# jolideco/jolideco

Hardware: AMD Instinct MI355X
Metric: MAP iters/sec at 2048x2048, 8-obs joint fit (higher is better)
Workload: dtype f32; 1 GPU; c3: 2048x2048, 8 observations (Gaussian PSFs sigma = 1.5 + 0.25 i on 6 x 17x17 + 2 x 33x33, varying exposure/background), GMM patch prior 8x8 stride 4 K=128, joint fit, Adam lr 0.1; global_observations=8, conv_method=separable

## Files before the change

### jolideco_amd/csrc/gmm_screen.hip

```cpp
#include "gmm_internal.h"

namespace jd {

struct __attribute__((packed, aligned(4))) F4U {
  float x, y, z, w;
};

__global__ __launch_bounds__(256) void gmm_stage_kernel(GmmStageArgs a) {
  use_device_shift(a);
  if (a.pcount && blockIdx.x == 0 && threadIdx.x == 0) *a.dense_count = 0;
  const int lane = threadIdx.x & 63;
  const int tile = blockIdx.x * 4 + (threadIdx.x >> 6);
  if (tile >= a.n_tiles) return;
  const int h = lane >> 5, c = lane & 31;
  const int n = a.n_begin + 32 * tile + c;
  const bool valid = n < a.n_end;
  const int py = valid ? n / a.nPx : 0, px = valid ? n - (n / a.nPx) * a.nPx : 0;
  const int x0 = px * a.stride - a.shift_x;
  const int xb = x0 < 0 ? x0 + a.W : x0;
  const bool straight = xb + 7 < a.W;
  float x[32];
#pragma unroll
  for (int s = 0; s < 4; ++s) {
    const float* row = a.flux + (size_t)wrap(py * a.stride + 2 * s + h - a.shift_y, a.H) * a.W;
// ... 192 lines not shown
    pL[p] = -INFINITY;
    pq[p] = 0.f;
    pc[p] = 0;
    okm[p] = __ballot(pok[p]);
  }

  ScreenFrags f0, f1;
  f32x16 acc[2][2][2];
  auto issue_pair = [&](f32x16 (&buf)[2][2], const ScreenFrags& f, int p) {
#pragma unroll
    for (int u = 0; u < 2; ++u) {
      mfma_screen(buf[u], f, xf[2 * p + u]);
    }
  };
  constexpr int KSTEP = KSPLIT ? 4 : 1;
  const int kk0 = KSPLIT ? wave : 0;
  struct KConst {
    int k;
    float ck, ef, sk2, mn, ack;
  };
  auto fetch_consts = [&](int pos) {
    KConst r;
    if (KC_LDS) {
      r.k = kc_k[pos];
      const float4 c4 = kc_f[pos];
      r.ck = c4.x, r.ef = c4.y, r.sk2 = c4.z, r.mn = c4.w, r.ack = kc_a[pos];
    } else {
      r.k = a.korder[pos];
      r.ck = a.const_k[r.k], r.ef = a.efro_k[r.k], r.sk2 = a.sk2_k[r.k], r.mn = a.mnorm_k[r.k];
      r.ack = fmaf(1e-6f, fabsf(r.ck), 1e-30f);
    }
    return r;
  };
  auto clamp_pos = [&](int pos) { return pos < a.K ? pos : (kk0 < a.K ? kk0 : 0); };
  auto fetch_k = [&](int pos) { return KC_LDS ? kc_k[pos] : a.korder[pos]; };
  KConst cur = fetch_consts(clamp_pos(kk0));
  KConst nxt = fetch_consts(clamp_pos(kk0 + KSTEP));
  load_frags16(f0, af, __builtin_amdgcn_readfirstlane(cur.k));
  load_frags16(f1, af, __builtin_amdgcn_readfirstlane(nxt.k));
  issue_pair(acc[0], f0, 0);
  int k_ahead_next = fetch_k(clamp_pos(kk0 + 2 * KSTEP));
  auto component = [&](ScreenFrags& fa, const ScreenFrags& fb, int kk, auto phase, bool live) {
    constexpr int PHASE = decltype(phase)::value;
    const int k = __builtin_amdgcn_readfirstlane(cur.k);
    const float ck = cur.ck, ef = cur.ef, sk2 = cur.sk2, mn = cur.mn;
    const float ack = cur.ack;
    const int k_ahead = k_ahead_next;
    k_ahead_next = fetch_k(clamp_pos(kk + 3 * KSTEP));
    cur = nxt;
    nxt = fetch_consts(clamp_pos(kk + 2 * KSTEP));
    unsigned long long m0 = 0ull, m1 = 0ull;
    float u0 = 0.f, u1 = 0.f;
    if (NP == 2) {
      issue_pair(acc[1], fa, 1);
      load_frags16(fa, af, __builtin_amdgcn_readfirstlane(k_ahead));
      screen_finish_pair<LSE>(acc[0][0], acc[0][1], ck, ack, mn, ef, pxn[0], ps2[0] * sk2, pok[0], pL[0], pq[0], pc[0], keep,
                              m0, u0, live ? okm[0] : 0ull, live);
      issue_pair(acc[0], fb, 0);
      screen_finish_pair<LSE>(acc[1][0], acc[1][1], ck, ack, mn, ef, pxn[NP - 1], ps2[NP - 1] * sk2, pok[NP - 1], pL[NP - 1],
                              pq[NP - 1], pc[NP - 1], keep, m1, u1, live ? okm[NP - 1] : 0ull, live);
    } else {
      load_frags16(fa, af, __builtin_amdgcn_readfirstlane(k_ahead));
      issue_pair(acc[1 - PHASE], fb, 0);
      screen_finish_pair<LSE>(acc[PHASE][0], acc[PHASE][1], ck, ack, mn, ef, pxn[0], ps2[0] * sk2, pok[0], pL[0], pq[0], pc[0],
                              keep, m0, u0, live ? okm[0] : 0ull, live);
    }
    if (NP == 2 && !LSE && !KSPLIT) {
#pragma unroll
      for (int i = 0; i < 12 * NP; ++i) {
        __builtin_amdgcn_sched_group_barrier(0x008, 1, 0);
        __builtin_amdgcn_sched_group_barrier(0x002, 8, 0);
      }
    }
    if (m0 | m1) {
      screen_emit(m0, u0, pn[0], k, lane, cnt_l, lb_n, lb_k, lb_ub, SCREEN_RB);
      if (NP == 2) screen_emit(m1, u1, pn[NP - 1], k, lane, cnt_l, lb_n, lb_k, lb_ub, SCREEN_RB);
      flush(false);
    }
  };
  for (int kk = kk0; kk < a.K; kk += 2 * KSTEP) {
    component(f0, f1, kk, std::integral_constant<int, 0>{}, true);
    component(f1, f0, kk + KSTEP, std::integral_constant<int, 1>{}, kk + KSTEP < a.K);
  }
  bool trouble = false;
#pragma unroll
  for (int p = 0; p < NP; ++p) {
    trouble = trouble || (pok[p] && !(pq[p] < 3.0e38f));
    if (LSE && pc[p] > keep && pn[p] < a.n_end) a.dense_mark[pn[p]] = 1;
    if (KSPLIT)
      st_L[wave * (NT * 32) + (2 * p + h) * 32 + c] = pL[p];
    else if (pn[p] < a.n_end)
      a.lfinal[pn[p]] = pL[p];
  }
  if (KSPLIT) {
    __syncthreads();
    for (int i = threadIdx.x; i < NT * 32; i += 256)
      if (base + i < a.n_end)
        a.lfinal[base + i] = fmaxf(fmaxf(st_L[i], st_L[NT * 32 + i]), fmaxf(st_L[2 * NT * 32 + i], st_L[3 * NT * 32 + i]));
  }
  flush(true);
  if (lane == 0) a.seg_cnt[wave_global] = cnt < SCREEN_CAP ? cnt : SCREEN_CAP;
  if (__ballot(trouble) != 0ull || cnt > SCREEN_CAP) {
    if (lane == 0) __hip_atomic_store(a.flag, a.gen, __ATOMIC_RELAXED, __HIP_MEMORY_SCOPE_AGENT);
  }
  if (CLOCK) {
    __syncthreads();
    if (threadIdx.x == 0 && (int)blockIdx.x < a.clock_cap) {
      a.clock_stamps[2 * blockIdx.x] = __builtin_amdgcn_s_memtime() - clock_t0;
      a.clock_stamps[2 * blockIdx.x + 1] = __builtin_amdgcn_s_memrealtime() - clock_r0;
    }
  }
}

#ifdef JD_EXACT_STAMPS
#define EXACT_STAMP(i)                                                              \
  do {                                                                              \
    __builtin_amdgcn_sched_barrier(0);                                              \
    const unsigned long long t_ = __builtin_amdgcn_s_memtime();                     \
    __builtin_amdgcn_sched_barrier(0);                                              \
    if (lane == 0) a.stamps[(size_t)grp * 8 + (i)] = t_;                            \
  } while (0)
#else
#define EXACT_STAMP(i) do {} while (0)
#endif

constexpr int EXACT_PITCH = 68;
constexpr int EXACT_DRAW = 1;
constexpr int EXACT_OFF_LDS = 1025;

template <bool TRI>
__global__ __launch_bounds__(256) void gmm_exact_kernel(GmmExactArgs a) {
  use_device_shift(a);
  if (*a.flag == a.gen) return;
  __shared__ __attribute__((aligned(16))) float stage[4][32 * EXACT_PITCH];
  const int lane = threadIdx.x & 63, wave = threadIdx.x >> 6;
  const int g = lane >> 4, n16 = lane & 15;
  const int wave_global = blockIdx.x * 4 + wave;
  const int n_waves = gridDim.x * 4;
  const int n_groups = a.offsets[a.K] >> 5;
  float* st = stage[wave];
  (void)n_waves, (void)wave_global;
  __shared__ int s_off[EXACT_OFF_LDS];
  __shared__ int s_next;
  const bool off_lds = a.K + 1 <= EXACT_OFF_LDS;
  const int per_block = (n_groups + (int)gridDim.x - 1) / (int)gridDim.x;
  const int b_begin = (int)blockIdx.x * per_block, b_end = b_begin + per_block < n_groups ? b_begin + per_block : n_groups;
  if (threadIdx.x == 0) s_next = b_begin;
  if (off_lds)
    for (int i = threadIdx.x; i <= a.K; i += 256) s_off[i] = a.offsets[i];
  __syncthreads();
  auto offset_of = [&](int kk) { return off_lds ? s_off[kk] : a.offsets[kk]; };
  int k = -1;
  float ck = 0.f;
  float4 A[4][4], M[4];
  for (;;) {
    int g_begin = 0;
    if (lane == 0) g_begin = atomicAdd(&s_next, EXACT_DRAW);
    g_begin = __builtin_amdgcn_readfirstlane(g_begin);
    if (g_begin >= b_end) break;
    const int g_end = g_begin + EXACT_DRAW < b_end ? g_begin + EXACT_DRAW : b_end;
  for (int grp = g_begin; grp < g_end; ++grp) {
    EXACT_STAMP(0);
    int kg = k;
    if (kg < 0 || offset_of(kg) > 32 * grp || offset_of(kg + 1) <= 32 * grp) {
      int lo = 0, hi = a.K;
      while (hi - lo > 1) {
        const int mid = (lo + hi) >> 1;
        if (offset_of(mid) <= 32 * grp) lo = mid; else hi = mid;
      }
      kg = lo;
    }
    if (kg != k) {
      k = kg;
      ck = a.const_k[k];
      const float4* ak = reinterpret_cast<const float4*>(a.afrag) + (size_t)k * (AFRAG_FLOATS / 4) + lane;
      const float4* mk = reinterpret_cast<const float4*>(a.mfrag) + (size_t)k * 16 + g;
#pragma unroll
      for (int jb = 0; jb < 4; ++jb) {
        M[jb] = mk[jb * 4];
#pragma unroll
        for (int st4 = 0; st4 < 4; ++st4)
          if (!TRI || st4 <= jb) A[jb][st4] = ak[(jb * 4 + st4) * 64];
      }
    }
    const int nvalid = a.counts[k] - (32 * grp - offset_of(k));
#ifdef JD_EXACT_STAMPS
    if (lane == 0) a.stamps[(size_t)grp * 8 + 7] = (unsigned long long)((nvalid << 8) | (k & 255));
    { float touch = A[0][0].x + M[0].x; asm volatile("" ::"v"(touch)); }
#endif
    EXACT_STAMP(1);
    {
      const int q = lane >> 1, hh = lane & 1;
      const bool have = q < nvalid;
      const int n = have ? a.order_n[32 * grp + q] : 0;
      const int py = n / a.nPx, px = n - py * a.nPx;
      const int x0 = px * a.stride + 4 * hh - a.shift_x;
      const bool straight = x0 >= 0 && x0 + 3 < a.W;
      const int xw[4] = {wrap(x0, a.W), wrap(x0 + 1, a.W), wrap(x0 + 2, a.W), wrap(x0 + 3, a.W)};
      float4 rows[8];
#pragma unroll
      for (int r = 0; r < 8; ++r) {
        const float* row = a.flux + (size_t)wrap(py * a.stride + r - a.shift_y, a.H) * a.W;
        if (straight) {
          const F4U v = *reinterpret_cast<const F4U*>(row + x0);
          rows[r] = make_float4(v.x, v.y, v.z, v.w);
        } else {
          rows[r] = make_float4(row[xw[0]], row[xw[1]], row[xw[2]], row[xw[3]]);
        }
      }
#pragma unroll
      for (int r = 0; r < 8; ++r) *reinterpret_cast<float4*>(st + q * EXACT_PITCH + 8 * r + 4 * hh) = rows[r];
    }
    EXACT_STAMP(2);
    int n[2];
    bool valid[2];
    float x[2][16];
#pragma unroll
    for (int nb = 0; nb < 2; ++nb) {
      const int q = 16 * nb + n16;
      valid[nb] = q < nvalid;
      n[nb] = valid[nb] ? a.order_n[32 * grp + q] : 0;
#pragma unroll
      for (int s4 = 0; s4 < 16; ++s4) x[nb][s4] = valid[nb] ? st[q * EXACT_PITCH + 4 * s4 + g] : 0.f;
      const float mean = patch_mean_groups(x[nb]);
#pragma unroll
      for (int s4 = 0; s4 < 16; ++s4) x[nb][s4] -= mean;
    }
#ifdef JD_EXACT_STAMPS
    { float touch = x[0][0] + x[1][15]; asm volatile("" ::"v"(touch)); }
#endif
    EXACT_STAMP(3);
    f32x4 y[4][2];
#pragma unroll
    for (int jb = 0; jb < 4; ++jb) {
      y[jb][0] = y[jb][1] = f32x4{M[jb].x, M[jb].y, M[jb].z, M[jb].w};
#pragma unroll
      for (int st4 = 0; st4 < 4; ++st4) {
        if (TRI && st4 > jb) continue;
#pragma unroll
        for (int e = 0; e < 4; ++e)
#pragma unroll
          for (int nb = 0; nb < 2; ++nb)
            y[jb][nb] = __builtin_amdgcn_mfma_f32_16x16x4f32(f4_get(A[jb][st4], e), x[nb][4 * st4 + e], y[jb][nb], 0, 0, 0);
      }
    }
#ifdef JD_EXACT_STAMPS
    { float touch = y[3][1][3] + y[0][0][0]; asm volatile("" ::"v"(touch)); }
#endif
    EXACT_STAMP(4);
#pragma unroll
    for (int nb = 0; nb < 2; ++nb) {
      const float l = fmaf(-0.5f, sum_lane_groups(sum_squares(y, nb)), ck);
      const int tie = a.grec ? 32 * grp + 16 * nb + n16 : k;
      if (a.lrec) {
        if (g == 0 && valid[nb]) a.lrec[32 * grp + 16 * nb + n16] = l;
      } else if (g == 0 && valid[nb] && l > -INFINITY) {
        atomicMax(a.best + n[nb], best_key(l, tie));
      }
    }
    EXACT_STAMP(5);
    if (a.grec) {
      float* rows[2] = {a.grec + (size_t)(32 * grp + n16) * D, a.grec + (size_t)(32 * grp + 16 + n16) * D};
      patch_gradient_rows<TRI>(y, a.gfrag, k, lane, valid, rows);
    }
#ifdef JD_EXACT_STAMPS
    __builtin_amdgcn_s_waitcnt(0);
#endif
    EXACT_STAMP(6);
  }
  }
}

constexpr int BEST_CHUNK = 1024;

__global__ __launch_bounds__(256) void gmm_best_kernel(GmmBestArgs a) {
  use_device_shift(a.fb);
  __shared__ double red[4];
  const int base = a.n_begin + blockIdx.x * BEST_CHUNK;
  const bool slots = a.winner && *a.flag != a.gen;
  double local = 0.0;
  unsigned long long keys[BEST_CHUNK / 256];
#pragma unroll
  for (int i = 0; i < BEST_CHUNK / 256; ++i) {
    const int n = base + i * 256 + threadIdx.x;
    keys[i] = a.best[n < a.n_end ? n : a.n_end - 1];
  }
  if (slots && !a.argmax_out) {
#pragma unroll
    for (int i = 0; i < BEST_CHUNK / 256; ++i) {
      const int n = base + i * 256 + threadIdx.x;
      if (n < a.n_end) {
        const unsigned long long key = keys[i];
        const bool ok = key != 0ull;
        const float v = best_value(key);
        a.winner[n] = ok && v > -INFINITY ? best_component(key) : -1;
        if (ok) local += (double)v;
      }
    }
  } else
#pragma unroll
  for (int i = 0; i < BEST_CHUNK / 256; ++i) {
    const int n = base + i * 256 + threadIdx.x;
    if (n < a.n_end) {
      const unsigned long long key = keys[i];
      const bool ok = key != 0ull;
      const float v = best_value(key);
      int k = ok ? best_component(key) : -1;
      if (slots) {
        const int slot = ok && v > -INFINITY ? k : -1;
        a.winner[n] = slot;
        if (a.argmax_out) k = ok ? (slot >= 0 ? a.rec_k[a.rec_order[slot]] : 0) : -1;
      } else if (a.argmax_fb) {
        a.argmax_fb[n] = k;
      }
      if (a.argmax_out) a.argmax_out[n] = k;
      if (ok) local += (double)v;
    }
  }
  local = wave_sum(local);
  if ((threadIdx.x & 63) == 0) red[threadIdx.x >> 6] = local;
  __syncthreads();
  if (a.fb.gpatch && !slots && a.winner) {
    __syncthreads();
    const int grp0 = blockIdx.x * (BEST_CHUNK / 32);
    const int n_groups = (a.n_end - a.n_begin + 31) >> 5;
    const int grp1 = grp0 + BEST_CHUNK / 32 < n_groups ? grp0 + BEST_CHUNK / 32 : n_groups;
    bwd_fallback_groups<true>(a.fb, grp0 + (threadIdx.x >> 6), grp1, 4);
  }
  __shared__ int last;
  if (threadIdx.x == 0) {
    a.partials[blockIdx.x] = (red[0] + red[1]) + (red[2] + red[3]);
    __threadfence();
    last = atomicAdd(a.ticket, 1) == (int)gridDim.x - 1 ? 1 : 0;
  }
  __syncthreads();
  if (!last) return;
  __threadfence();
  __shared__ double smem[4];
  double acc = 0.0;
  for (int i = threadIdx.x; i < (int)gridDim.x; i += 256) {
    const unsigned long long bits = __hip_atomic_load(reinterpret_cast<const unsigned long long*>(a.partials + i),
                                                      __ATOMIC_RELAXED, __HIP_MEMORY_SCOPE_AGENT);
    acc += __builtin_bit_cast(double, bits);
  }
  const double total = block_sum<256>(acc, smem);
  if (threadIdx.x == 0) {
    double v = a.scale * total;
    if (a.accumulate) v += (double)a.value_out[0];
    a.value_out[0] = (float)v;
    *a.ticket = 0;
    if (a.host_stats) {
      a.host_stats[1] = *a.flag == a.gen ? 1 : 0;
      a.host_stats[2] = *a.slots_used;
      a.host_stats[3] = a.n_end - a.n_begin;
      __threadfence_system();
      a.host_stats[0] = a.gen;
    }
  }
}

constexpr int LSE_ROWS = 32;

__global__ __launch_bounds__(256) void gmm_lse_combine_kernel(GmmLseCombineArgs a) {
  __shared__ int s_slot[16][LSE_ROWS];
  __shared__ float s_l[16][LSE_ROWS];
  if (*a.flag == a.gen) return;
  const int grp = threadIdx.x >> 4, part = threadIdx.x & 15;
  const int n = a.n_begin + (int)blockIdx.x * 16 + grp;
  const bool live = n < a.n_end && a.mark[n < a.n_end ? n : a.n_begin] == 0;
  int c = live ? a.pcount[n] : 0;
  if (c > a.rows) c = a.rows;
  int slot[2];
  float l[2];
#pragma unroll
  for (int u = 0; u < 2; ++u) {
    const int j = part + 16 * u;
    slot[u] = j < c ? a.ptab[(size_t)n * a.rows + j] : 0x7fffffff;
    l[u] = j < c ? a.lrec[slot[u]] : -INFINITY;
  }
  int rank[2] = {0, 0};
  for (int j = 0; j < c; ++j) {
    const int other = __shfl(j < 16 ? slot[0] : slot[1], (threadIdx.x & 48) + (j & 15), 64);
    rank[0] += other < slot[0] ? 1 : 0;
    rank[1] += other < slot[1] ? 1 : 0;
  }
#pragma unroll
  for (int u = 0; u < 2; ++u)
    if (part + 16 * u < c) s_slot[grp][rank[u]] = slot[u], s_l[grp][rank[u]] = l[u];
  float m = fmaxf(l[0], l[1]);
#pragma unroll
  for (int o = 8; o >= 1; o >>= 1) m = fmaxf(m, __shfl_xor(m, o, 64));
  __syncthreads();
  float4 G = make_float4(0.f, 0.f, 0.f, 0.f);
  float S = 0.f;
  for (int r = 0; r < c; ++r) {
    const float e = expf(s_l[grp][r] - m);
    const float4 row = reinterpret_cast<const float4*>(a.grec + (size_t)s_slot[grp][r] * D)[part];
    S += e;
    G.x = fmaf(e, row.x, G.x), G.y = fmaf(e, row.y, G.y), G.z = fmaf(e, row.z, G.z), G.w = fmaf(e, row.w, G.w);
  }
  if (live) {
    const float inv = c > 0 ? 1.f / S : 0.f;
    reinterpret_cast<float4*>(a.gpatch + (size_t)(n - a.n_begin) * D)[part] = make_float4(G.x * inv, G.y * inv, G.z * inv, G.w * inv);
  }
  if (part == 0 && live) a.vpatch[n] = c > 0 ? m + logf(S) : 0.f;
}

__global__ __launch_bounds__(256) void gmm_lse_list_kernel(const int* mark, int n_begin, int n_end, const int* flag, int gen,
                                                           int32_t* list, int* count) {
  __shared__ int wave_cnt[4][4];
  __shared__ int base;
  if (*flag == gen) return;
  const int lane = threadIdx.x & 63, wave = threadIdx.x >> 6;
  const int first = n_begin + (int)blockIdx.x * 1024;
  bool marked[4];
  int rank[4];
#pragma unroll
  for (int i = 0; i < 4; ++i) {
    const int n = first + i * 256 + (int)threadIdx.x;
    marked[i] = n < n_end && mark[n] != 0;
    const unsigned long long b = __ballot(marked[i]);
    rank[i] = __popcll(b & ((1ull << lane) - 1ull));
    if (lane == 0) wave_cnt[i][wave] = __popcll(b);
  }
  __syncthreads();
  if (threadIdx.x == 0) {
    int total = 0;
#pragma unroll
    for (int i = 0; i < 4; ++i)
#pragma unroll
      for (int w = 0; w < 4; ++w) {
        const int c = wave_cnt[i][w];
        wave_cnt[i][w] = total;
        total += c;
      }
    base = total ? atomicAdd(count, total) : 0;
  }
  __syncthreads();
#pragma unroll
  for (int i = 0; i < 4; ++i)
    if (marked[i]) list[base + wave_cnt[i][wave] + rank[i]] = first + i * 256 + (int)threadIdx.x;
}

__global__ __launch_bounds__(256) void gmm_lse_value_kernel(const float* vpatch, const int* mark, int n_begin, int n_end,
                                                            double* partials, int* marked) {
  __shared__ double red[4];
  __shared__ int redm[4];
  const int base = n_begin + (int)blockIdx.x * 1024;
  double local = 0.0;
  int cnt = 0;
#pragma unroll
  for (int i = 0; i < 4; ++i) {
    const int n = base + i * 256 + (int)threadIdx.x;
    const bool marked = n < n_end && mark[n] != 0;
    if (n < n_end) local += (double)vpatch[n];
    cnt += __popcll(__ballot(marked));
  }
  local = wave_sum(local);
  if ((threadIdx.x & 63) == 0) red[threadIdx.x >> 6] = local, redm[threadIdx.x >> 6] = cnt;
  __syncthreads();
  if (threadIdx.x == 0) {
    partials[blockIdx.x] = (red[0] + red[1]) + (red[2] + red[3]);
    marked[blockIdx.x] = (redm[0] + redm[1]) + (redm[2] + redm[3]);
  }
}

__global__ __launch_bounds__(256) void gmm_lse_finalize_kernel(const double* partials, const int* marked, int count,
                                                               const int* flag, int gen, double scale, float* value_out,
                                                               int accumulate, int* host_stats, const int* slots_used,
                                                               int patches) {
  __shared__ double smem[4];
  __shared__ int smem_i[4];
  double acc = 0.0;
  int cnt = 0;
  for (int i = threadIdx.x; i < count; i += 256) acc += partials[i], cnt += marked[i];
  const double total = block_sum<256>(acc, smem);
  for (int o = 32; o >= 1; o >>= 1) cnt += __shfl_xor(cnt, o, 64);
  if ((threadIdx.x & 63) == 0) smem_i[threadIdx.x >> 6] = cnt;
  __syncthreads();
  if (threadIdx.x == 0) {
    double v = scale * total;
    if (accumulate) v += (double)value_out[0];
    value_out[0] = (float)v;
    if (host_stats) {
      const int n_marked = (smem_i[0] + smem_i[1]) + (smem_i[2] + smem_i[3]);
      host_stats[1] = *flag == gen ? 1 : (5 * (long)n_marked > 3 * (long)patches ? 2 : 0);
      host_stats[2] = *slots_used;
      host_stats[3] = patches;
      __threadfence_system();
      host_stats[0] = gen;
    }
  }
}

#ifdef JD_EXACT_STAMPS
static int launch_exact_stamped(jd_gmm* g, GmmExactArgs& ex, size_t slots, hipStream_t s) {
  static unsigned long long* stamps_dev = nullptr;
  static size_t stamps_cap = 0;
  const size_t max_groups = slots / 32 + g->K + 8;
  if (stamps_cap < max_groups) {
    if (stamps_dev) (void)hipFree(stamps_dev);
    JD_HIP(hipMalloc(&stamps_dev, max_groups * 8 * sizeof(unsigned long long)));
    stamps_cap = max_groups;
  }
  ex.stamps = stamps_dev;
  {
    ProfScope stage(JD_KERNEL_GMM_EXACT, s);
    gmm_exact_kernel<true><<<(unsigned)(g->n_cu * 3), 256, 0, s>>>(ex);
  }
  JD_LAUNCH_CHECK();
  if (!opt_is_set(OPT_GMM_SCREEN_DEBUG)) return JD_OK;
  JD_HIP(hipStreamSynchronize(s));
  int total_slots = 0;
  JD_HIP(hipMemcpy(&total_slots, ex.offsets + g->K, sizeof(int), hipMemcpyDeviceToHost));
  const int n_groups = total_slots >> 5;
  std::vector<unsigned long long> st((size_t)n_groups * 8);
  JD_HIP(hipMemcpy(st.data(), stamps_dev, st.size() * sizeof(unsigned long long), hipMemcpyDeviceToHost));
  const char* names[6] = {"bucket + fragments", "indices + patch rows -> LDS", "LDS read-back + mean", "first product (80 MFMAs)",
                          "value epilogue + atomicMax", "second product + gradient rows"};
  double sum[6] = {0};
  std::vector<double> per[6];
  unsigned long long t_min = ~0ull, t_max = 0;
  for (int gi = 0; gi < n_groups; ++gi) {
    const unsigned long long* t = &st[(size_t)gi * 8];
    for (int ph = 0; ph < 6; ++ph) {
      const double dt = (double)(t[ph + 1] - t[ph]);
      sum[ph] += dt;
      per[ph].push_back(dt);
    }
    t_min = t[0] < t_min ? t[0] : t_min, t_max = t[6] > t_max ? t[6] : t_max;
  }
  fprintf(stderr, "[jd exact stamps] %d groups of 32 records, first stamp to last stamp %.0f shader cycles\n", n_groups,
          (double)(t_max - t_min));
  double total = 0;
  for (int ph = 0; ph < 6; ++ph) total += sum[ph];
  for (int ph = 0; ph < 6; ++ph) {
    std::sort(per[ph].begin(), per[ph].end());
    const size_t m = per[ph].size();
    fprintf(stderr, "[jd exact stamps] %-34s mean %8.0f cycles (%4.1f %%)  q10 %7.0f  q50 %7.0f  q90 %7.0f  q99 %7.0f\n", names[ph],
            sum[ph] / n_groups, 100.0 * sum[ph] / total, per[ph][m / 10], per[ph][m / 2], per[ph][m * 9 / 10], per[ph][m * 99 / 100]);
  }
  fprintf(stderr, "[jd exact stamps] per group %.0f cycles; groups per wave %.2f; waves %d\n", total / n_groups,
          (double)n_groups / (double)(g->n_cu * 12), g->n_cu * 12);
  return JD_OK;
}
#endif

static int launch_exact(jd_gmm* g, GmmExactArgs& ex, size_t slots, hipStream_t s) {
#ifdef JD_EXACT_STAMPS
  return launch_exact_stamped(g, ex, slots, s);
#else
  {
    ProfScope stage(JD_KERNEL_GMM_EXACT, s);
    gmm_exact_kernel<true><<<(unsigned)(g->n_cu * 3), 256, 0, s>>>(ex);
  }
  JD_LAUNCH_CHECK();
  return JD_OK;
#endif
}

int screened_forward(jd_gmm* g, const GmmFwdArgs& a, hipStream_t s, int* n_partials, bool fused, int32_t* fallback_argmax,
                     double value_scale, float* value_out, int accumulate_value, bool lse) {
  jd_gmm::Screen& sn = g->screen;
  const long n = a.n_end - a.n_begin;
  bool ksplit = (n + SCREEN_T * 32 * 4 - 1) / (SCREEN_T * 32 * 4) < g->n_cu;
  if (opt_is_set(OPT_GMM_KSPLIT)) ksplit = opt_value(OPT_GMM_KSPLIT, 0) != 0;
  constexpr int T = SCREEN_T;
  const unsigned blocks = (unsigned)(ksplit ? (n + T * 32 - 1) / (T * 32) : ((n + T * 32 - 1) / (T * 32) + 3) / 4);
  const size_t n_seg = (size_t)blocks * 4;
  const size_t slots = n_seg * SCREEN_CAP;
  const size_t bucket_slots = slots + 32 * (size_t)g->K;
  JD_REQUIRE(bucket_slots < (size_t)1 << 31, "jd_gmm_prior_fwd_bwd: too many patches for the screened path");
  int rc;
  if ((rc = sn.best.reserve((size_t)a.n_end))) return rc;
  if ((rc = sn.lfinal.reserve((size_t)a.n_end))) return rc;
  if ((rc = sn.rec.reserve(3 * slots))) return rc;
  if ((rc = sn.rec_order.reserve(bucket_slots))) return rc;
  if ((rc = sn.rec_order_n.reserve(bucket_slots))) return rc;
  if ((rc = sn.seg_cnt.reserve(n_seg))) return rc;
  if ((rc = g->dense.partials.reserve((size_t)((n + 31) / 32 + 4)))) return rc;
  int32_t* rec_n = sn.rec.ptr;
  int32_t* rec_k = sn.rec.ptr + slots;
  float* rec_ub = reinterpret_cast<float*>(sn.rec.ptr + 2 * slots);
  int* flag = sn.ctl.ptr;
  sn.gen = sn.gen % (1 << 30) + 1;
  if (a.shift_dev) JD_HIP(hipMemsetAsync(flag, 0, sizeof(int), s));
  if (fused && g->fused.stats.host) {
    volatile int* hs = g->fused.stats.host;
    const int seen = hs[0];
    if (seen != g->fused.stats_seen_gen && seen > 0) {
      const long used = hs[2], patches = hs[3];
      if (patches > 0 && (hs[1] != 0 || used - 32L * g->K > (long)(0.6 * g->fused.rows_per_patch * (double)patches)) &&
          g->fused.rows_per_patch < 32)
        g->fused.rows_per_patch *= 2;
      g->fused.stats_seen_gen = seen;
    }
  }
  const size_t grec_rows = fused ? (size_t)g->fused.rows_per_patch * (size_t)n + 32 * (size_t)g->K : 0;
  if (fused) {
    if ((rc = g->fused.grec.reserve(grec_rows * D))) return rc;
    if ((rc = g->fused.winner.reserve((size_t)a.n_end))) return rc;
  }
  const unsigned combine_blocks = (unsigned)((n + 15) / 16), value_blocks = (unsigned)((n + 1023) / 1024);
  if (lse) {
    if ((rc = g->lse.lrec.reserve(bucket_slots))) return rc;
    if ((rc = g->lse.pcount.reserve((size_t)a.n_end))) return rc;
    if ((rc = g->lse.dense_mark.reserve((size_t)a.n_end))) return rc;
    if ((rc = g->lse.vpatch.reserve((size_t)a.n_end))) return rc;
    if ((rc = g->lse.ptab.reserve((size_t)a.n_end * LSE_ROWS))) return rc;
    if ((rc = g->lse.partials.reserve((size_t)value_blocks))) return rc;
    if ((rc = g->lse.marked.reserve((size_t)value_blocks))) return rc;
    if ((rc = g->lse.dense_list.reserve((size_t)n + 1))) return rc;
  }

  const size_t n_tiles = (size_t)blocks * (ksplit ? T : 4 * T);
  if ((rc = sn.xfrag.reserve(n_tiles * 4 * 64))) return rc;
  if ((rc = sn.xstat.reserve(2 * n_tiles * 32))) return rc;
  if ((rc = sn.xok.reserve(n_tiles * 32))) return rc;

  unsigned chunks = (unsigned)n_seg;
  unsigned max_blocks = std::max<unsigned>(2u * g->n_cu, (1u << 20) / (unsigned)g->K);
  if (opt_value(OPT_GMM_SORT_BLOCKS, 0) > 0) max_blocks = (unsigned)opt_value(OPT_GMM_SORT_BLOCKS, 0);
  if (chunks > max_blocks) chunks = max_blocks;
  if ((rc = g->sort.blk_counts.reserve((size_t)chunks * g->K))) return rc;
  const bool kc_lds = g->K <= SCREEN_KC_MAX && !opt_is_set(OPT_GMM_SCREEN_NO_LDS_CONSTS);
  int* const dense_mark = lse ? g->lse.dense_mark.ptr : nullptr;
  int* const dense_count = lse ? reinterpret_cast<int*>(g->lse.dense_list.ptr) : nullptr;

  ProfScope prof(JD_KERNEL_GMM_FWD, s);
  GmmStageArgs stg{};
  set_patch_grid(stg, a);
  stg.flux = a.flux, stg.n_begin = a.n_begin, stg.n_end = a.n_end, stg.n_tiles = (int)n_tiles;
  stg.pcount = lse ? g->lse.pcount.ptr : nullptr, stg.dense_mark = dense_mark, stg.dense_count = dense_count;
  stg.xfrag = sn.xfrag.ptr, stg.xn = sn.xstat.ptr, stg.xs2 = sn.xstat.ptr + n_tiles * 32, stg.ok = sn.xok.ptr, stg.best = sn.best.ptr;
  GmmScreenArgs sc{};
  set_patch_grid(sc, a);
  sc.flux = a.flux, sc.K = a.K, sc.n_begin = a.n_begin, sc.n_end = a.n_end;
  sc.xfrag = sn.xfrag.ptr, sc.xn = stg.xn, sc.xs2 = stg.xs2, sc.ok = sn.xok.ptr;
  sc.afrag16 = sn.afrag16.ptr, sc.const_k = g->dense.const_k.ptr, sc.efro_k = sn.efro_k.ptr, sc.sk2_k = sn.sk2_k.ptr;
  sc.mnorm_k = sn.mnorm_k.ptr, sc.korder = sn.korder.ptr;
  sc.lfinal = sn.lfinal.ptr, sc.rec_n = rec_n, sc.rec_k = rec_k, sc.rec_ub = rec_ub;
  sc.seg_cnt = sn.seg_cnt.ptr, sc.flag = flag, sc.gen = sn.gen, sc.dense_mark = dense_mark;
  {
    ProfScope stage(JD_KERNEL_GMM_STAGE, s);
    gmm_stage_kernel<<<(unsigned)((n_tiles + 3) / 4), 256, 0, s>>>(stg);
  }
  JD_LAUNCH_CHECK();
  {
    ProfScope stage(JD_KERNEL_GMM_SCREEN, s);
    if (lse && ksplit)
      gmm_screen_kernel<2, true, true, true><<<blocks, 256, 0, s>>>(sc);
    else if (lse)
      gmm_screen_kernel<2, false, true, true><<<blocks, 256, 0, s>>>(sc);
    else if (ksplit && kc_lds)
      gmm_screen_kernel<2, true, true><<<blocks, 256, 0, s>>>(sc);
    else if (ksplit)
      gmm_screen_kernel<2, true, false><<<blocks, 256, 0, s>>>(sc);
    else if (kc_lds && sn.clock_stamps.ptr) {
      sc.clock_stamps = sn.clock_stamps.ptr, sc.clock_cap = SCREEN_CLOCK_CAP;
      gmm_screen_kernel<2, false, true, false, true><<<blocks, 256, 0, s>>>(sc);
    } else if (kc_lds)
      gmm_screen_kernel<2, false, true><<<blocks, 256, 0, s>>>(sc);
    else
      gmm_screen_kernel<2, false, false><<<blocks, 256, 0, s>>>(sc);
  }
  JD_LAUNCH_CHECK();

  GmmBucketArgs bk{};
  bk.argmax = rec_k, bk.n_begin = 0, bk.n_end = (int)slots, bk.K = g->K;
  bk.counts = sn.ctl.ptr + 1, bk.offsets = sn.ctl.ptr + 1 + 2 * g->K;
  bk.order = sn.rec_order.ptr, bk.order_n = sn.rec_order_n.ptr, bk.gpatch = nullptr;
  bk.seg_cnt = sn.seg_cnt.ptr, bk.seg_cap = SCREEN_CAP, bk.rec_n = rec_n, bk.rec_ub = rec_ub, bk.lfinal = sn.lfinal.ptr;
  bk.chunk = SCREEN_CAP;
  bk.korder = g->K <= KORDER_MAX_K ? sn.korder.ptr : nullptr;
  if (fused) bk.flag = flag, bk.gen = sn.gen, bk.slot_cap = (int)std::min<size_t>(grec_rows, (size_t)INT32_MAX);
  if (lse) bk.margin = LSE_MARGIN, bk.pcount = g->lse.pcount.ptr, bk.ptab = g->lse.ptab.ptr, bk.ptab_rows = LSE_ROWS, bk.dense_mark = dense_mark;
  bk.blk_counts = g->sort.blk_counts.ptr;
  {
    ProfScope stage(JD_KERNEL_GMM_SORT, s);
    launch_bucket_sort(bk, chunks, s);
  }
  JD_LAUNCH_CHECK();

  GmmExactArgs ex{};
  set_patch_grid(ex, a);
  ex.flux = a.flux, ex.afrag = g->dense.afrag.ptr, ex.mfrag = g->dense.mfrag.ptr, ex.const_k = g->dense.const_k.ptr;
  ex.order_n = sn.rec_order_n.ptr, ex.counts = bk.counts, ex.offsets = bk.offsets, ex.flag = flag, ex.gen = sn.gen;
  ex.gfrag = g->dense.gfrag.ptr, ex.grec = fused ? g->fused.grec.ptr : nullptr, ex.lrec = lse ? g->lse.lrec.ptr : nullptr;
  ex.best = sn.best.ptr, ex.K = g->K;
  if ((rc = launch_exact(g, ex, slots, s))) return rc;

  if (lse) {
    GmmBwdLseArgs b{};
    set_patch_grid(b, a);
    b.flux = a.flux, b.afrag = g->dense.afrag.ptr, b.mfrag = g->dense.mfrag.ptr, b.gfrag = g->dense.gfrag.ptr, b.const_k = g->dense.const_k.ptr;
    b.partials = g->dense.partials.ptr, b.gpatch = g->dense.gpatch.ptr, b.K = g->K;
    b.n_begin = a.n_begin, b.n_end = a.n_end, b.run_flag = flag, b.run_gen = sn.gen;
    b.mark = dense_mark, b.vpatch = g->lse.vpatch.ptr;
    b.list = g->lse.dense_list.ptr + 1, b.list_count = dense_count;
    gmm_lse_list_kernel<<<value_blocks, 256, 0, s>>>(dense_mark, a.n_begin, a.n_end, flag, sn.gen, g->lse.dense_list.ptr + 1, dense_count);
    JD_LAUNCH_CHECK();
    long bblocks = ((n + 31) / 32 + 2 * 4 - 1) / (2 * 4);
    if (bblocks > g->n_cu) bblocks = g->n_cu;
    launch_bwd_lse(b, true, (unsigned)bblocks, s);
    JD_LAUNCH_CHECK();
    GmmLseCombineArgs cb{};
    cb.pcount = g->lse.pcount.ptr, cb.ptab = g->lse.ptab.ptr, cb.rows = LSE_ROWS, cb.lrec = g->lse.lrec.ptr, cb.grec = g->fused.grec.ptr;
// ... 84 lines not shown
```

### jolideco_amd/csrc/kernels.h

```cpp
#pragma once
#include <vector>
#include "jd_common.h"

namespace jd {

struct PoissonArgs {
  const float* conv[JD_MAX_COMPONENTS];
  float* g[JD_MAX_COMPONENTS];
  const float* background;
  const float* counts;
  float* npred_out;
  double* partials;
  int n_comp, H, W, Hp, Wp, oy, ox;
  float eps, inv_n;
  int write_grad;
  int up;
  const float* log_bkg_norm;
  double* partials_b;
};

struct PoissonMixedArgs {
  const float* conv[JD_MAX_COMPONENTS];
  float* g[JD_MAX_COMPONENTS];
  int up[JD_MAX_COMPONENTS], Wp[JD_MAX_COMPONENTS], oy[JD_MAX_COMPONENTS], ox[JD_MAX_COMPONENTS];
  const float* background;
  const float* counts;
  float* npred_out;
  double* partials;
  int n_comp, Hd, Wd;
  float eps, inv_n;
  int write_grad;
};
int launch_poisson_mixed(const PoissonMixedArgs& a, int* n_partials, hipStream_t stream);
int poisson_mixed_max_partials(int Hd, int Wd);

int launch_pad_mul(const float* image, const float* scale, float* padded, int H, int W, int Hp, int Wp,
                   hipStream_t stream);
int launch_cmul(float2* spec, const float2* khat, size_t n, bool conj, hipStream_t stream);
int launch_poisson_fused(const PoissonArgs& a, int* n_partials, hipStream_t stream);
int launch_poisson_pooled(const PoissonArgs& a, int* n_partials, hipStream_t stream);
int poisson_fused_max_partials(int Hp, int Wp);
int launch_adjoint_epilogue(const float* corr, const float* scale, float* grad, int H, int W, int Hp,
                            int Wp, int oy, int ox, float coef, int accumulate, hipStream_t stream);
int launch_crop(const float* padded, float* out, int H, int W, int Wp, int oy, int ox, hipStream_t stream);

int launch_shift_fwd(const float* in, float* out, int H, int W, const float* shift_xy, float scale, hipStream_t stream);
int launch_shift_bwd(const float* in, const float* gs, float* grad_in, int accumulate, int H, int W,
                     const float* shift_xy, float scale, double* partials, int* n_blocks, hipStream_t stream);
int shift_bwd_max_blocks(int H, int W);
int shift_bwd_route(int H, int W);
struct FftBatch;
int launch_shift_bwd_batch(const float* in, const FftBatch* batch, int n_datasets, float* grad_in, int accumulate, int H, int W,
                           float scale, double* partials, size_t partials_stride, int* n_blocks, hipStream_t stream);
int launch_finalize_multi_batch(const double* partials, size_t stride, int n_blocks, int n_datasets, float* const* out,
                                hipStream_t stream);
int launch_finalize_multi(const double* partials, int n_blocks, int n_out, double scale, float* out, int accumulate,
                          hipStream_t stream);

enum { JD_CONV_FFT = 0, JD_CONV_DIRECT = 1, JD_CONV_SEPARABLE = 2 };
bool direct_conv_supported(int kh, int kw);
bool direct_conv_split_supported(int kh, int kw);
size_t direct_conv_fragment_floats(int kh, int kw, int split);
int launch_toeplitz_fragments(const float* psf, float* afrag_fwd, float* afrag_adj, int kh, int kw, int split,
                              hipStream_t stream);
int launch_direct_conv(const float* in, const float* in_scale, const float* afrag, float* out, const float* out_scale,
                       int H, int W, int kh, int kw, int oy, int ox, int adjoint, float coef, int accumulate, int split,
                       hipStream_t stream);
int direct_conv_tiles(int H, int W);
void direct_conv_route(int W, int kw, int ox, int split, int* route4);
int launch_direct_conv_poisson(const float* in, const float* in_scale, const float* afrag, float* g_out, int H, int W,
                               int kh, int kw, int oy, int ox, const float* background, const float* counts,
                               float* npred_out, double* partials, float eps, float inv_n, int write_grad,
                               int* n_partials, int split, hipStream_t stream);

enum JdOption {
  OPT_SEP_NO_ALIAS, OPT_SEP_FWD_MIN_LDS, OPT_SEP_ADJ_MIN_LDS, OPT_SEP_INTERLEAVE, OPT_SEP_NO_FUSION, OPT_SEP_WALK,
  OPT_SEP_WALK_COLS, OPT_SEP_WALK_ROWS, OPT_SEP_WALK_ADJ_COLS, OPT_SEP_WALK_ADJ_ROWS, OPT_DIRECT_FP32,
  OPT_CONV_BLOCKS_PER_CU, OPT_POISSON_ROWS, OPT_GMM_NO_HOST_STATS, OPT_GMM_BLOCK_TILES, OPT_GMM_DENSE, OPT_GMM_KSPLIT,
  OPT_GMM_SCREEN_NO_LDS_CONSTS, OPT_GMM_SCREEN_DEBUG, OPT_GMM_SCREEN, OPT_GMM_FUSED_BWD,
  OPT_GMM_GATHER_TILED, OPT_GMM_LSE_SCREEN, OPT_SEP_JOINT, OPT_SEP_JOINT_ROWS, OPT_SEP_JOINT_CHUNK,
  OPT_SEP_WALK_ADJ_ALL, OPT_SEP_WALK_COST33, OPT_SEP_WALK_ROWS33, OPT_SEP_NO_TRIM, OPT_SEP_WALK_ADJ_ROWS33,
  OPT_SEP_WALK_ADJ33, OPT_FFT_NATIVE, OPT_DIRECT_AUTO_ALL, OPT_FFT_BATCH, OPT_FFT_TINY, OPT_FFT_POOL_IO, OPT_GMM_SORT_BLOCKS, OPT_GMM_GATHER_PRELOAD,
  OPT_SEP_ADJ_ADDENDS, OPT_SEP_WALK_CHAIN, OPT_SEP_WALK_ADJ_CHAIN, OPT_COUNT
};
bool opt_is_set(int id);
int opt_value(int id, int unset_value);

constexpr int SEP_MAX_K = 68, SEP_MAX_RANK = 3, SEP_MAX_BATCH = 16;
struct SepGeom {
  int khp, kwp;
  int oy0, ox0;
  int shiftx;
  int rpairs;
  int pitch;
};
SepGeom sep_geom(int kh, int kw, int oy, int ox, bool adjoint);
struct SepOpInfo {
  int rank = 0;
  int ulo[2] = {0, 0}, uhi[2] = {0, 0}, vlo[2] = {0, 0}, vhi[2] = {0, 0};
};
inline unsigned sep_pack_support(int ulo, int uhi, int vlo, int vhi) {
  return (unsigned)ulo | (unsigned)uhi << 8 | (unsigned)vlo << 16 | (unsigned)vhi << 24;
}
void sep_register_operator(const void* op_dev, const SepOpInfo& info);
void sep_forget_operator(const void* op_dev);
int sep_operator_rank(const void* op_dev);
bool sep_operator_info(const void* op_dev, SepOpInfo* info);
constexpr double SEP_DEFAULT_TOL = 3e-7;
bool sep_conv_supported(int kh, int kw);
size_t sep_conv_operator_floats();
int sep_factorize(const float* psf_host, int kh, int kw, double tol, std::vector<double>* u, std::vector<double>* v);
int sep_build_operator(const float* psf_host, int kh, int kw, int oy, int ox, double tol, std::vector<float>* op,
                       SepOpInfo* info = nullptr);
struct SepLossFold {
  const double* partials;
  int count;
  double scale, offset;
  float* out;
};
int launch_sep_conv(const float* in, const float* in_scale, const float* op, float* out, const float* out_scale, int H,
                    int W, int kh, int kw, int oy, int ox, int adjoint, float coef, int accumulate, hipStream_t stream,
                    const SepLossFold* fold = nullptr, int* fold_done = nullptr);
int sep_guard_check(int** guard_dev);
int sep_conv_tiles(int H, int W);
constexpr int SEP_BATCH_MAX_COMP = 4;
struct SepBatchTable {
  const float* scale[SEP_MAX_BATCH * SEP_BATCH_MAX_COMP];
  const float* op[SEP_MAX_BATCH * SEP_BATCH_MAX_COMP];
  float* g[SEP_MAX_BATCH * SEP_BATCH_MAX_COMP];
  const float* bkg[SEP_MAX_BATCH];
  const float* cnt[SEP_MAX_BATCH];
  float* loss_out[SEP_MAX_BATCH];
  float loss_offset[SEP_MAX_BATCH];
  int order[SEP_MAX_BATCH];
  int n17;
  unsigned long long frame33;
  float* addend[SEP_MAX_BATCH];
};
constexpr int SEP_ADDEND_MAX = 4;
int sep_addend_split(int n, const SepBatchTable& table, int H, int W, int kh, int kw, int oy, int ox);
void walk_batch_order(SepBatchTable& table, int n, int n_comp, int kh, int kw, int oy, int ox);
int launch_sep_conv_poisson_batch(int n, int n_comp, const float* const* flux, const SepBatchTable& table,
                                  const SepBatchTable* table_dev, int H, int W, int kh, int kw, int oy, int ox,
                                  double* partials, float eps, float inv_n, int write_grad, int* n_partials,
                                  hipStream_t stream);
int launch_sep_conv_adjoint_batch(int n, int n_comp, int comp, const SepBatchTable& table, const SepBatchTable* table_dev,
                                  float* grad, int H, int W, int kh, int kw, int oy, int ox, float coef, int accumulate,
                                  hipStream_t stream, const double* fin_partials = nullptr, double fin_scale = 0.0,
                                  int fin_count = 0, int* fin_done = nullptr, int addend_first = -1,
                                  hipStream_t stream2 = nullptr, const hipEvent_t* fork_join = nullptr);
bool sep_batch_is_mixed(int n, int n_comp, const SepBatchTable& table, int H, int W, int kh, int kw, int oy, int ox);

constexpr int JD_WALK_NOT_TAKEN = 1;
bool walk_takes_launch(int H, int W, int n_datasets, int kh, int kw, int oy, int ox);
int walk_operator_frame(const float* op, int kh, int kw, int oy, int ox);
int walk_info_frame(const SepOpInfo& info, int kh, int kw, int oy, int ox);
int walk_conv(const float* in, const float* in_scale, const float* op, float* out, const float* out_scale, int H, int W,
              int kh, int kw, int oy, int ox, int adjoint, float coef, int accumulate, hipStream_t stream);
int walk_conv_poisson(const float* in, const float* in_scale, const float* op, float* g_out, int H, int W, int kh, int kw,
                      int oy, int ox, const float* background, const float* counts, float* npred_out, double* partials,
                      float eps, float inv_n, int write_grad, int* n_partials, hipStream_t stream);
int walk_conv_poisson_batch(int n, const float* flux, const SepBatchTable& table, const SepBatchTable* table_dev, int H,
                            int W, int kh, int kw, int oy, int ox, double* partials, float eps, float inv_n,
                            int write_grad, int* n_partials, hipStream_t stream);
int walk_joint_step(int n, const float* flux, const SepBatchTable& table, const SepBatchTable* table_dev, float* grad, int H,
                    int W, int kh, int kw, int oy, int ox, double* partials, float eps, float inv_n, float coef,
                    int accumulate, int* n_partials, hipStream_t stream);
int walk_conv_poisson_batch_multi(int n, int n_comp, const float* const* flux, const SepBatchTable& table,
                                  const SepBatchTable* table_dev, int H, int W, int kh, int kw, int oy, int ox,
                                  double* partials, float eps, float inv_n, int write_grad, int* n_partials,
                                  hipStream_t stream);
int walk_conv_adjoint_batch(int n, int n_comp, int comp, const SepBatchTable& table, const SepBatchTable* table_dev,
                            float* grad, int H, int W, int kh, int kw, int oy, int ox, float coef, int accumulate,
                            hipStream_t stream, const double* fin_partials, double fin_scale, int fin_count, int* fin_done,
                            int addend_first = -1, hipStream_t stream2 = nullptr, const hipEvent_t* fork_join = nullptr);
int walk_conv_adjoint_batch_all(int n, int n_comp, const SepBatchTable& table, const SepBatchTable* table_dev,
                                float* const* grads, int H, int W, int kh, int kw, int oy, int ox, float coef, int accumulate,
                                hipStream_t stream, const double* fin_partials, double fin_scale, int fin_count,
                                int* fin_done);
int launch_finalize_rows(const double* partials, int n, int n_out, double scale, const float* offset_host,
                         float* const* out, hipStream_t stream);
int launch_sep_conv_poisson(const float* in, const float* in_scale, const float* op, float* g_out, int H, int W, int kh,
                            int kw, int oy, int ox, const float* background, const float* counts, float* npred_out,
                            double* partials, float eps, float inv_n, int write_grad, int* n_partials,
                            hipStream_t stream);

struct FftNative {
  int H = 0, W = 0, kh = 0, kw = 0, oy = 0, ox = 0, Hh = 0, Nx = 0, Ny = 0;
  float2* spec = nullptr;
  float2* work = nullptr;
  float2* tw_x = nullptr;
  float2* tw_y = nullptr;
};
bool fftn_supported(int H, int W, int kh, int kw);
int fftn_create(FftNative* n, int H, int W, int kh, int kw);
void fftn_destroy(FftNative* n);
size_t fftn_spectrum_elements(const FftNative& n);
int fftn_spectrum(const FftNative& n, const float* psf, float2* khat, hipStream_t stream);
int fftn_conv(const FftNative& n, const float* in, const float* in_scale, const float2* khat, float* out, const float* out_scale,
              int adjoint, float coef, int accumulate, hipStream_t stream);
int fftn_poisson_step(const FftNative& n, const float* flux, const float* exposure, const float2* khat, const float* background,
                      const float* counts, double* partials, int* n_partials, float eps, float inv_n, float* grad, float coef,
                      int accumulate, hipStream_t stream, double loss_scale, double loss_offset, float* loss_out);

constexpr int FFT_MAX_BATCH = 16;
struct FftBatch {
  int n;
  const float* exposure[FFT_MAX_BATCH];
  const float2* khat[FFT_MAX_BATCH];
  const float* background[FFT_MAX_BATCH];
  const float* counts[FFT_MAX_BATCH];
  float2* spec[FFT_MAX_BATCH];
  float2* work[FFT_MAX_BATCH];
  float* loss_out[FFT_MAX_BATCH];
  float loss_offset[FFT_MAX_BATCH];
  const float* shift_xy[FFT_MAX_BATCH];
  const float* log_bkg_norm[FFT_MAX_BATCH];
  float* grad_shift_xy[FFT_MAX_BATCH];
  float* grad_log_bkg_norm[FFT_MAX_BATCH];
  float* gshift[FFT_MAX_BATCH];
};
int fftn_poisson_step_batch(const FftNative& n, int nd, const FftBatch* batch_dev, const float* flux, double* partials, float eps,
                            float inv_n, float* grad, float coef, int accumulate, hipStream_t stream, double loss_scale);
int fftn_poisson_step_pooled_batch(const FftNative& n, int upsampling, int nd, const FftBatch* batch_dev, const FftBatch& host,
                                   const float* flux, double* partials, double* partials_b, float eps, float inv_n, float* grad,
                                   double* partials_shift, float coef, int accumulate, hipStream_t stream, double loss_scale,
                                   double norm_grad_scale, int sequential);
bool fftn_pooled_supported(const FftNative& n, int upsampling);
void fftn_step_route(const FftNative& n, int upsampling, int per_launch, int* route6);
int fftn_fft_route(const FftNative& n, int n_datasets, int* route7);
int fftn_poisson_step_pooled(const FftNative& n, int upsampling, const float* flux, const float* exposure, const float2* khat,
                             const float* background, const float* counts, const float* log_bkg_norm, double* partials,
                             double* partials_b, float eps, float inv_n, float* target, float coef, int accumulate,
                             hipStream_t stream, double loss_scale, double loss_offset, float* loss_out, double norm_grad_scale,
                             float* norm_grad_out, const float* shift_xy, float shift_scale);

// ... 11 lines not shown
```

### jolideco_amd/csrc/options.hip

```cpp
#include <atomic>
#include <climits>
#include <cstdlib>
#include <cstring>

#include "jd_common.h"
#include "kernels.h"

namespace jd {

namespace {
struct OptionSlot {
  const char* name;
  std::atomic<int> value;
};
OptionSlot g_options[OPT_COUNT] = {
    {"JD_SEP_NO_ALIAS", {INT_MIN}},      {"JD_SEP_FWD_MIN_LDS", {INT_MIN}},  {"JD_SEP_ADJ_MIN_LDS", {INT_MIN}},
    {"JD_SEP_INTERLEAVE", {INT_MIN}},    {"JD_SEP_NO_FUSION", {INT_MIN}},    {"JD_SEP_WALK", {INT_MIN}},
    {"JD_SEP_WALK_COLS", {INT_MIN}},     {"JD_SEP_WALK_ROWS", {INT_MIN}},    {"JD_SEP_WALK_ADJ_COLS", {INT_MIN}},
    {"JD_SEP_WALK_ADJ_ROWS", {INT_MIN}}, {"JD_DIRECT_FP32", {INT_MIN}},      {"JD_CONV_BLOCKS_PER_CU", {INT_MIN}},
    {"JD_POISSON_ROWS", {INT_MIN}},      {"JD_GMM_NO_HOST_STATS", {INT_MIN}}, {"JD_GMM_BLOCK_TILES", {INT_MIN}},
    {"JD_GMM_DENSE", {INT_MIN}},         {"JD_GMM_KSPLIT", {INT_MIN}},
    {"JD_GMM_SCREEN_NO_LDS_CONSTS", {INT_MIN}}, {"JD_GMM_SCREEN_DEBUG", {INT_MIN}}, {"JD_GMM_SCREEN", {INT_MIN}},
    {"JD_GMM_FUSED_BWD", {INT_MIN}},     {"JD_GMM_GATHER_TILED", {INT_MIN}}, {"JD_GMM_LSE_SCREEN", {INT_MIN}},
    {"JD_SEP_JOINT", {INT_MIN}},         {"JD_SEP_JOINT_ROWS", {INT_MIN}},
    {"JD_SEP_JOINT_CHUNK", {INT_MIN}},   {"JD_SEP_WALK_ADJ_ALL", {INT_MIN}}, {"JD_SEP_WALK_COST33", {INT_MIN}},
    {"JD_SEP_WALK_ROWS33", {INT_MIN}},   {"JD_SEP_NO_TRIM", {INT_MIN}},      {"JD_SEP_WALK_ADJ_ROWS33", {INT_MIN}},
    {"JD_SEP_WALK_ADJ33", {INT_MIN}},    {"JD_FFT_NATIVE", {INT_MIN}},
    {"JD_DIRECT_AUTO_ALL", {INT_MIN}},
    {"JD_FFT_BATCH", {INT_MIN}},
    {"JD_FFT_TINY", {INT_MIN}},
    {"JD_FFT_POOL_IO", {INT_MIN}},
    {"JD_GMM_SORT_BLOCKS", {INT_MIN}},
    {"JD_GMM_GATHER_PRELOAD", {INT_MIN}},
    {"JD_SEP_ADJ_ADDENDS", {INT_MIN}},
    {"JD_SEP_WALK_CHAIN", {INT_MIN}},
    {"JD_SEP_WALK_ADJ_CHAIN", {INT_MIN}},
};

int parse(const char* text) {
  char* end = nullptr;
  const long v = strtol(text, &end, 10);
  if (end == text) return 1;
  return v <= INT_MIN ? INT_MIN + 1 : v > INT_MAX ? INT_MAX : (int)v;
}

struct EnvInit {
  EnvInit() {
    for (auto& o : g_options)
      if (const char* env = getenv(o.name)) o.value.store(parse(env));
  }
} g_env_init;
}

bool opt_is_set(int id) { return g_options[id].value.load(std::memory_order_relaxed) != INT_MIN; }
int opt_value(int id, int unset_value) {
  const int v = g_options[id].value.load(std::memory_order_relaxed);
  return v == INT_MIN ? unset_value : v;
}

}

using namespace jd;

extern "C" int jd_set_option(const char* key, const char* value) {
  JD_REQUIRE(key, "jd_set_option: key is null");
  for (auto& o : g_options)
    if (strcmp(o.name, key) == 0) {
      o.value.store(value ? parse(value) : INT_MIN);
      return JD_OK;
    }
  return fail(JD_ERR_INVALID, "jd_set_option: unknown option '%s'", key);
}

extern "C" int jd_get_option(const char* key, int* is_set, int* value) {
  JD_REQUIRE(key && is_set && value, "jd_get_option: null argument");
  for (auto& o : g_options)
    if (strcmp(o.name, key) == 0) {
      const int v = o.value.load();
      *is_set = v != INT_MIN, *value = v == INT_MIN ? 0 : v;
      return JD_OK;
    }
  return fail(JD_ERR_INVALID, "jd_get_option: unknown option '%s'", key);
}
```

Measured before the change: 1870 iters/s.

## Stream GMM exact-kernel fragments per block and raise exact kernel occupancy

```diff
diff --git a/jolideco_amd/csrc/gmm_screen.hip b/jolideco_amd/csrc/gmm_screen.hip
--- a/jolideco_amd/csrc/gmm_screen.hip
+++ b/jolideco_amd/csrc/gmm_screen.hip
@@ -368,7 +368,14 @@
   auto offset_of = [&](int kk) { return off_lds ? s_off[kk] : a.offsets[kk]; };
   int k = -1;
   float ck = 0.f;
-  float4 A[4][4], M[4];
+  const float4* ak = nullptr;
+  const float4* mk = nullptr;
+  auto fragments = [&](int jb, float4& M, float4 (&A)[4]) {
+    M = mk[jb * 4];
+#pragma unroll
+    for (int st4 = 0; st4 < 4; ++st4)
+      if (!TRI || st4 <= jb) A[st4] = ak[(jb * 4 + st4) * 64];
+  };
   for (;;) {
     int g_begin = 0;
     if (lane == 0) g_begin = atomicAdd(&s_next, EXACT_DRAW);
@@ -389,45 +396,40 @@
     if (kg != k) {
       k = kg;
       ck = a.const_k[k];
-      const float4* ak = reinterpret_cast<const float4*>(a.afrag) + (size_t)k * (AFRAG_FLOATS / 4) + lane;
-      const float4* mk = reinterpret_cast<const float4*>(a.mfrag) + (size_t)k * 16 + g;
-#pragma unroll
-      for (int jb = 0; jb < 4; ++jb) {
-        M[jb] = mk[jb * 4];
-#pragma unroll
-        for (int st4 = 0; st4 < 4; ++st4)
-          if (!TRI || st4 <= jb) A[jb][st4] = ak[(jb * 4 + st4) * 64];
-      }
+      ak = reinterpret_cast<const float4*>(a.afrag) + (size_t)k * (AFRAG_FLOATS / 4) + lane;
+      mk = reinterpret_cast<const float4*>(a.mfrag) + (size_t)k * 16 + g;
     }
     const int nvalid = a.counts[k] - (32 * grp - offset_of(k));
 #ifdef JD_EXACT_STAMPS
     if (lane == 0) a.stamps[(size_t)grp * 8 + 7] = (unsigned long long)((nvalid << 8) | (k & 255));
-    { float touch = A[0][0].x + M[0].x; asm volatile("" ::"v"(touch)); }
 #endif
     EXACT_STAMP(1);
     {
       const int q = lane >> 1, hh = lane & 1;
       const bool have = q < nvalid;
-      const int n = have ? a.order_n[32 * grp + q] : 0;
+      const int n = a.order_n[32 * grp + (have ? q : 0)];
       const int py = n / a.nPx, px = n - py * a.nPx;
       const int x0 = px * a.stride + 4 * hh - a.shift_x;
       const bool straight = x0 >= 0 && x0 + 3 < a.W;
-      const int xw[4] = {wrap(x0, a.W), wrap(x0 + 1, a.W), wrap(x0 + 2, a.W), wrap(x0 + 3, a.W)};
+      const int xs = straight ? x0 : 0;
       float4 rows[8];
 #pragma unroll
-      for (int r = 0; r < 8; ++r) {
-        const float* row = a.flux + (size_t)wrap(py * a.stride + r - a.shift_y, a.H) * a.W;
-        if (straight) {
-          const F4U v = *reinterpret_cast<const F4U*>(row + x0);
-          rows[r] = make_float4(v.x, v.y, v.z, v.w);
-        } else {
-          rows[r] = make_float4(row[xw[0]], row[xw[1]], row[xw[2]], row[xw[3]]);
+      for (int r = 0; r < 8; ++r)
+        rows[r] = gld4u(a.flux + (size_t)wrap(py * a.stride + r - a.shift_y, a.H) * a.W + xs);
+      if (!straight) {
+        const int xw[4] = {wrap(x0, a.W), wrap(x0 + 1, a.W), wrap(x0 + 2, a.W), wrap(x0 + 3, a.W)};
+#pragma unroll
+        for (int r = 0; r < 8; ++r) {
+          const float* row = a.flux + (size_t)wrap(py * a.stride + r - a.shift_y, a.H) * a.W;
+          rows[r] = make_float4(gld(row + xw[0]), gld(row + xw[1]), gld(row + xw[2]), gld(row + xw[3]));
         }
       }
 #pragma unroll
       for (int r = 0; r < 8; ++r) *reinterpret_cast<float4*>(st + q * EXACT_PITCH + 8 * r + 4 * hh) = rows[r];
     }
     EXACT_STAMP(2);
+    float4 Mf[2], Af[2][4];
+    fragments(0, Mf[0], Af[0]);
     int n[2];
     bool valid[2];
     float x[2][16];
@@ -435,7 +437,7 @@
     for (int nb = 0; nb < 2; ++nb) {
       const int q = 16 * nb + n16;
       valid[nb] = q < nvalid;
-      n[nb] = valid[nb] ? a.order_n[32 * grp + q] : 0;
+      n[nb] = a.order_n[32 * grp + (valid[nb] ? q : 0)];
 #pragma unroll
       for (int s4 = 0; s4 < 16; ++s4) x[nb][s4] = valid[nb] ? st[q * EXACT_PITCH + 4 * s4 + g] : 0.f;
       const float mean = patch_mean_groups(x[nb]);
@@ -449,7 +451,10 @@
     f32x4 y[4][2];
 #pragma unroll
     for (int jb = 0; jb < 4; ++jb) {
-      y[jb][0] = y[jb][1] = f32x4{M[jb].x, M[jb].y, M[jb].z, M[jb].w};
+      const float4& M = Mf[jb & 1];
+      const float4(&A)[4] = Af[jb & 1];
+      if (jb < 3) fragments(jb + 1, Mf[(jb + 1) & 1], Af[(jb + 1) & 1]);
+      y[jb][0] = y[jb][1] = f32x4{M.x, M.y, M.z, M.w};
 #pragma unroll
       for (int st4 = 0; st4 < 4; ++st4) {
         if (TRI && st4 > jb) continue;
@@ -457,7 +462,7 @@
         for (int e = 0; e < 4; ++e)
 #pragma unroll
           for (int nb = 0; nb < 2; ++nb)
-            y[jb][nb] = __builtin_amdgcn_mfma_f32_16x16x4f32(f4_get(A[jb][st4], e), x[nb][4 * st4 + e], y[jb][nb], 0, 0, 0);
+            y[jb][nb] = __builtin_amdgcn_mfma_f32_16x16x4f32(f4_get(A[st4], e), x[nb][4 * st4 + e], y[jb][nb], 0, 0, 0);
       }
     }
 #ifdef JD_EXACT_STAMPS
@@ -709,6 +714,11 @@
   }
 }
 
+static unsigned exact_blocks(const jd_gmm* g) {
+  const int per_cu = opt_value(OPT_GMM_EXACT_BLOCKS, 4);
+  return (unsigned)(g->n_cu * (per_cu < 1 ? 1 : per_cu > 8 ? 8 : per_cu));
+}
+
 #ifdef JD_EXACT_STAMPS
 static int launch_exact_stamped(jd_gmm* g, GmmExactArgs& ex, size_t slots, hipStream_t s) {
   static unsigned long long* stamps_dev = nullptr;
@@ -722,7 +732,7 @@
   ex.stamps = stamps_dev;
   {
     ProfScope stage(JD_KERNEL_GMM_EXACT, s);
-    gmm_exact_kernel<true><<<(unsigned)(g->n_cu * 3), 256, 0, s>>>(ex);
+    gmm_exact_kernel<true><<<exact_blocks(g), 256, 0, s>>>(ex);
   }
   JD_LAUNCH_CHECK();
   if (!opt_is_set(OPT_GMM_SCREEN_DEBUG)) return JD_OK;
@@ -732,7 +742,7 @@
   const int n_groups = total_slots >> 5;
   std::vector<unsigned long long> st((size_t)n_groups * 8);
   JD_HIP(hipMemcpy(st.data(), stamps_dev, st.size() * sizeof(unsigned long long), hipMemcpyDeviceToHost));
-  const char* names[6] = {"bucket + fragments", "indices + patch rows -> LDS", "LDS read-back + mean", "first product (80 MFMAs)",
+  const char* names[6] = {"bucket", "indices + patch rows -> LDS", "LDS read-back + mean", "fragments + first product (80 MFMAs)",
                           "value epilogue + atomicMax", "second product + gradient rows"};
   double sum[6] = {0};
   std::vector<double> per[6];
@@ -757,7 +767,7 @@
             sum[ph] / n_groups, 100.0 * sum[ph] / total, per[ph][m / 10], per[ph][m / 2], per[ph][m * 9 / 10], per[ph][m * 99 / 100]);
   }
   fprintf(stderr, "[jd exact stamps] per group %.0f cycles; groups per wave %.2f; waves %d\n", total / n_groups,
-          (double)n_groups / (double)(g->n_cu * 12), g->n_cu * 12);
+          (double)n_groups / (double)(exact_blocks(g) * 4), (int)(exact_blocks(g) * 4));
   return JD_OK;
 }
 #endif
@@ -768,7 +778,7 @@
 #else
   {
     ProfScope stage(JD_KERNEL_GMM_EXACT, s);
-    gmm_exact_kernel<true><<<(unsigned)(g->n_cu * 3), 256, 0, s>>>(ex);
+    gmm_exact_kernel<true><<<exact_blocks(g), 256, 0, s>>>(ex);
   }
   JD_LAUNCH_CHECK();
   return JD_OK;
diff --git a/jolideco_amd/csrc/kernels.h b/jolideco_amd/csrc/kernels.h
--- a/jolideco_amd/csrc/kernels.h
+++ b/jolideco_amd/csrc/kernels.h
@@ -81,7 +81,7 @@
   OPT_GMM_GATHER_TILED, OPT_GMM_LSE_SCREEN, OPT_SEP_JOINT, OPT_SEP_JOINT_ROWS, OPT_SEP_JOINT_CHUNK,
   OPT_SEP_WALK_ADJ_ALL, OPT_SEP_WALK_COST33, OPT_SEP_WALK_ROWS33, OPT_SEP_NO_TRIM, OPT_SEP_WALK_ADJ_ROWS33,
   OPT_SEP_WALK_ADJ33, OPT_FFT_NATIVE, OPT_DIRECT_AUTO_ALL, OPT_FFT_BATCH, OPT_FFT_TINY, OPT_FFT_POOL_IO, OPT_GMM_SORT_BLOCKS, OPT_GMM_GATHER_PRELOAD,
-  OPT_SEP_ADJ_ADDENDS, OPT_SEP_WALK_CHAIN, OPT_SEP_WALK_ADJ_CHAIN, OPT_COUNT
+  OPT_SEP_ADJ_ADDENDS, OPT_SEP_WALK_CHAIN, OPT_SEP_WALK_ADJ_CHAIN, OPT_GMM_EXACT_BLOCKS, OPT_COUNT
 };
 bool opt_is_set(int id);
 int opt_value(int id, int unset_value);
diff --git a/jolideco_amd/csrc/options.hip b/jolideco_amd/csrc/options.hip
--- a/jolideco_amd/csrc/options.hip
+++ b/jolideco_amd/csrc/options.hip
@@ -35,6 +35,7 @@
     {"JD_SEP_ADJ_ADDENDS", {INT_MIN}},
     {"JD_SEP_WALK_CHAIN", {INT_MIN}},
     {"JD_SEP_WALK_ADJ_CHAIN", {INT_MIN}},
+    {"JD_GMM_EXACT_BLOCKS", {INT_MIN}},
 };
 
 int parse(const char* text) {
```

New measurement: 1881 iters/s (median of 6 runs). No clear change (+0.6%).
